# NOAA-GFDL/GRTCODE

Measured on AMD Instinct MI355X. Metric: columns/sec (60-layer, 1 cm⁻¹ LBL, LW+SW), higher is better.
Workload: dtype f64

## Files before the change

### grtcode_amd/csrc/grt_kernels.h

```cpp
#ifndef GRT_KERNELS_H_
#define GRT_KERNELS_H_

#include <stddef.h>
#include <stdint.h>

#ifdef __cplusplus
extern "C" {
#endif

#define GRT_MAX_ISO 18
#define GRT_MAX_SLOTS 53
#define GRT_MAX_TABLES 32

typedef struct GrtLineStore
{
    uint64_t n;
    double const *v0;
    double const *s0;
    float const *yair;
    float const *yself;
    float const *en;
    float const *nexp;
    float const *delta;
    uint8_t const *iso;
// ... 33 lines not shown
    GrtLineStore lines;
    GrtColumnLayout lay;
    double const *colstate;
    double const *tables;
    double const *h2o_tables;
    double w0, wres;
    uint64_t nw;
    int ncol;
    double *tau;
    uint64_t tau_col_stride;
    int tile;
    int nslice;
    int fast;
    float *gmom;
    uint64_t gmom_stride;
    int halo;
    int rcap;
    int tree_levels;
    int mom_terms;
    int profile_tag;
    int near_block;
    int deterministic;
    unsigned long long *probe;
    int direct_near;
    int tile_phase, tile_nphase;
    uint32_t const *tile_ranges;
    int lean;
    uint32_t const *tile_items;
    uint32_t n_items;
    GrtTableSpans spans;
    int *radius_table;
    int skip_tables;
    int narrow;
} GrtGasOpticsArgs;

typedef struct GrtContinua
{
    double const *colstate;
    uint64_t stride, off_cont, off_h2o;
    double const *tables;
    double const *h2o_tables;
    int num_tables, has_h2o_ctm;
    GrtTableSpans spans;
} GrtContinua;
int grt_launch_add_continua(void *stream, GrtContinua const *c, int num_layers, int ncol, uint64_t nw,
                            double *tau_gas, uint64_t col_stride);


int grt_launch_gas_optics(void *stream, GrtGasOpticsArgs const *a);
enum { GRT_TAG_FAR_OFFSET = 5 };
int grt_profile_begin(void *stream, int tag);
void grt_profile_end(void *stream, int slot);
int grt_launch_gas_optics_mp(void *stream, GrtGasOpticsArgs const *a);
int grt_gas_optics_mp_shape(GrtGasOpticsArgs const *a);
int grt_gas_optics_lean_shape(GrtGasOpticsArgs const *a);
void grt_work_order(unsigned nb, unsigned per_group, unsigned ngroups, unsigned b, unsigned *group, unsigned *rem);
int grt_tree_gather_by_wave(long long fsteps);
uint64_t grt_gas_optics_moment_floats(uint64_t nw, int levels, int terms);
double grt_gas_optics_moment_separation(int terms);

typedef struct GrtSweepBins
{
    double w0, wres;
    uint64_t num_wpoints, n;
    int ppb, do_interp, do_last_interp;
    double const *w;
    double *tau;
    uint64_t const *l, *r;
} GrtSweepBins;
int grt_launch_sweep_sort(void *stream, uint64_t n, int num_layers, double const *v0, double shift_max,
                          double const *lay, double const *prep, double *sorted);
int grt_launch_sweep(void *stream, int method, uint64_t n, int num_layers, double const *lines,
                     double const *ns, GrtSweepBins const *bins, double *tau);
int grt_launch_sweep_interpolate(void *stream, int num_layers, GrtSweepBins const *bins, double *tau);

int grt_launch_line_prep(void *stream, GrtGasOpticsArgs const *a, int col,
                         double *vnn, double *snn, double *gamma, double *alpha,
                         int64_t *win_s, int64_t *win_e);

int grt_launch_voigt_debug(void *stream, int fast, double w_start, uint64_t n, double wres, double center,
                           double gamma, double alpha, double *K_dev);

int grt_launch_voigt_points(void *stream, int variant, uint64_t n, double const *x_dev, double const *y_dev,
                            double *K_dev, int *cls_dev);

int grt_launch_device_math(void *stream, int op, uint64_t n, double const *a_dev, double *out0_dev, double *out1_dev);

int grt_launch_rayleigh(void *stream, int num_layers, double w0, double dw, uint64_t nw,
                        double const *n_layer_host, double *tau, double *omega, double *g);

typedef struct GrtOpticsPtrs { double const *tau[8]; double const *omega[8]; double const *g[8]; } GrtOpticsPtrs;
// ... 453 lines not shown
```

### grtcode_amd/csrc/hip/gas_optics_mp_dev.h

```cpp
#ifndef GRT_GAS_OPTICS_MP_DEV_H_
#define GRT_GAS_OPTICS_MP_DEV_H_
#include <type_traits>
#include "gas_optics_dev.h"

namespace {

constexpr int kMom = 8;
constexpr int kFarGradedMin = 64;
constexpr int kMomWide = 12;

__host__ __device__ inline double moment_separation(int terms)
{
    return terms == kMomWide ? 3.95 : 7.8;
}
constexpr size_t kLdsPerWorkgroup = 64*1024;
constexpr int kRcap = 12;
constexpr int kPowTable = 128;
constexpr int kCellLoop = 3;

template <int CTRL>
__device__ __forceinline__ float dpp_f(float v)
{
    int const b = __float_as_int(v);
    return __int_as_float(__builtin_amdgcn_update_dpp(0, b, CTRL, 0xf, 0xf, true));
// ... 133 lines not shown
    {
        float const keep = b1 ? x[i + 2] : x[i];
        float const send = b1 ? x[i] : x[i + 2];
        y[i] = keep + dpp_f<0x1B>(send);
    }
    float const keep = b0 ? y[1] : y[0];
    float const send = b0 ? y[0] : y[1];
    return keep + dpp_f<0xB1>(send);
}

constexpr int kRawCap = 128;
constexpr int kLeanListCap = 12;
constexpr int kLeanMaxP = 4;
constexpr int kLeanSlots = 16;
struct LeanTables
{
    float ps[kLeanSlots];
    float qn_m[kLeanSlots*GRT_MAX_ISO];
    float dop[kLeanSlots];
    float qn_e[kLeanSlots*GRT_MAX_ISO];
    float ptab[kPowTable];
    float p_ps[kLeanSlots];
};
static_assert(kLeanSlots*GRT_MAX_ISO > 255 && kLeanSlots*GRT_MAX_ISO + kPowTable > 255, "ps, dop and p_ps within reach of a paired read");
struct LeanRaw
{
    unsigned long long xl_mask[kWaves][kLeanListCap][kLeanMaxP];
    unsigned j[kWaves][kRawCap];
    float amp[kWaves][kRawCap];
    float delta[kWaves][kRawCap];
    unsigned idx[kWaves][kRawCap];
    unsigned xl_base[kWaves][kLeanListCap];
};

constexpr int kClasses = 3;
constexpr int kClassesSplit = 4;
constexpr int kMpQueue = 64;
constexpr int kMpQueueTree = 64;

template <int CAP, int NCLS>
struct MpQueue
{
    static constexpr int capacity = CAP;
    static constexpr int classes = NCLS;
    float amp[NCLS][kWaves][CAP];
    float xi[NCLS][kWaves][CAP];
    float y[NCLS][kWaves][CAP];
    unsigned short idx[NCLS][kWaves][CAP];
};
using MpQueueFlat = MpQueue<kMpQueue, kClassesSplit>;
using MpQueueTree = MpQueue<kMpQueueTree, kClassesSplit>;

__device__ __attribute__((noinline)) double exp_fp64_call(double x)
{
    return exp_fp64(x);
}

constexpr int binomial(int n, int k)
{
    int r = 1;
    for (int i = 1; i <= k; ++i)
    {
        r = r*(n - k + i)/i;
    }
    return r;
}
// ... 143 lines not shown
```

### grtcode_amd/csrc/hip/k_gas_optics_far.hip

```cpp
#include "gas_optics_mp_dev.h"

namespace {

__global__ __launch_bounds__(kBlock) void near_radius_kernel(GrtGasOpticsArgs a, long long fsteps_ll, int cell_shift, int ntiles)
{
    extern __shared__ __attribute__((aligned(16))) unsigned char smem[];
    double *ms_l = reinterpret_cast<double *>(smem);
    double *q_l = ms_l + 4*a.lay.num_slots;
    int const tid = threadIdx.x;
    int const layer = blockIdx.x, col = blockIdx.y;
    double const *cs = a.colstate + (uint64_t)col*a.lay.stride;
    double const *lay = cs + a.lay.off_lay + (uint64_t)layer*4;
    stage_column_state(a, cs, layer, ms_l, q_l, tid);
    __syncthreads();
    long long const nw = (long long)a.nw;
    for (int t = tid; t < ntiles; t += kBlock)
    {
        long long const c1 = ((long long)(t + 1) << cell_shift);
        bool um, cr;
        int const R = near_radius(a, lay, ms_l, (long long)t << cell_shift, c1 < nw ? c1 : nw, (int)fsteps_ll, &um, &cr);
        long long const F1 = c1 < nw ? c1 : nw;
        unsigned const tf = lean_tile_flags(a, lay, ms_l, (int)((long long)t << cell_shift), (int)F1, cr);
        a.radius_table[((uint64_t)col*a.lay.num_layers + layer)*ntiles + t] = R | (um ? 0x10000 : 0) | (cr ? 0x20000 : 0) | (int)(tf << kTileFlagsShift);
    }
}

__global__ __launch_bounds__(kBlock) void gas_optics_far_kernel(GrtGasOpticsArgs a, long long fsteps_ll, int cell_shift, int ncell)
{
    extern __shared__ __attribute__((aligned(16))) unsigned char smem[];
    int const fsteps = (int)fsteps_ll;
    double *acc = reinterpret_cast<double *>(smem);
    double *ms_l = acc + a.tile;
    double *q_l = ms_l + 4*a.lay.num_slots;
    float *mom = reinterpret_cast<float *>(q_l + GRT_MAX_ISO*a.lay.num_slots);
    float *invr = mom + (size_t)kMom*ncell;
    int *rtab = reinterpret_cast<int *>(invr + fsteps + 1);
    int const tid = threadIdx.x;
    int const layer = blockIdx.y, col = blockIdx.z;
    long long const nw = (long long)a.nw;
    long long const F0l = (long long)blockIdx.x*a.tile;
    long long const F1l = (F0l + a.tile < nw) ? F0l + a.tile : nw;
    int const F0 = (int)F0l, F1 = (int)F1l;
    double const *cs = a.colstate + (uint64_t)col*a.lay.stride;
    double const *lay = cs + a.lay.off_lay + (uint64_t)layer*4;
    double *out = a.tau + (uint64_t)col*a.tau_col_stride + (uint64_t)layer*a.nw;
    bool const own_radii = a.radius_table == nullptr || fsteps > kFarGradedMin;
    if (own_radii)
    {
        stage_column_state(a, cs, layer, ms_l, q_l, tid);
    }
    for (int i = tid; i <= fsteps; i += kBlock)
    {
        invr[i] = i > 0 ? 1.0f/(float)i : 0.f;
    }
    int const cell0 = F0 - fsteps;
    float const *gm = a.gmom + ((uint64_t)col*a.lay.num_layers + layer)*a.gmom_stride;
// ... 700 lines not shown
extern "C" size_t grt_far_lds_bytes(int tile, int ncell, int fsteps, int num_slots, int cell_shift)
{
    return far_lds_bytes(tile, ncell, fsteps, num_slots, cell_shift);
}

extern "C" size_t grt_tree_lds_bytes(int tile, int num_slots, int ntab)
{
    return tree_lds_bytes(tile, num_slots, ntab);
}

extern "C" int grt_tree_gather_tile(void)
{
    return tree_gather_tile();
}

extern "C" int grt_tree_gather_ntab(int tile, int halo)
{
    return tree_gather_ntab(tile, halo);
}

extern "C" int grt_tree_gather_by_wave(long long fsteps)
{
    return tree_gather_by_wave(fsteps) ? 1 : 0;
}

extern "C" int grt_launch_near_radius(void *stream, GrtGasOpticsArgs const *bp, long long fsteps, int shift)
{
    int const ntiles = (int)((bp->nw + ((uint64_t)1 << shift) - 1) >> shift);
    hipLaunchKernelGGL(near_radius_kernel, dim3(bp->lay.num_layers, bp->ncol), dim3(kBlock),
                       sizeof(double)*bp->lay.num_slots*(4 + GRT_MAX_ISO), (hipStream_t)stream, *bp, fsteps, shift, ntiles);
    return (int)hipGetLastError();
}

extern "C" int grt_launch_far_field(void *stream, GrtGasOpticsArgs const *bp, long long fsteps, int shift)
{
    hipStream_t const s = (hipStream_t)stream;
    GrtGasOpticsArgs b = *bp;
    if (b.tree_levels > 0)
    {
        int first_level = 1;
        while ((2 << (first_level - 1)) <= b.tile && first_level <= b.tree_levels) ++first_level;
        if (b.mom_terms == kMomWide)
        {
            launch_tree<kMomWide>(s, b, fsteps, shift, first_level);
        }
        else
        {
            launch_tree<kMom>(s, b, fsteps, shift, first_level);
        }
        return (int)hipGetLastError();
    }
    int const far_want = 512;
    int far_tile = b.tile;
    while (2*far_tile <= far_want && (uint64_t)far_tile < b.nw
           && far_lds_bytes(2*far_tile, 2*far_tile + 2*(int)fsteps, (int)fsteps, b.lay.num_slots, shift) <= kLdsPerWorkgroup)
    {
        far_tile *= 2;
    }
    b.tile = far_tile;
    unsigned const far_tiles = (unsigned)((b.nw + far_tile - 1)/far_tile);
    int const far_ncell = far_tile + 2*(int)fsteps;
    hipLaunchKernelGGL(gas_optics_far_kernel, dim3(far_tiles, b.lay.num_layers, b.ncol), dim3(kBlock),
                       far_lds_bytes(far_tile, far_ncell, (int)fsteps, b.lay.num_slots, shift), s, b, fsteps, shift, far_ncell);
    return (int)hipGetLastError();
}
```

### grtcode_amd/csrc/hip/k_gas_optics_mp.hip

```cpp
#include "gas_optics_mp_dev.h"

extern "C" size_t grt_far_lds_bytes(int tile, int ncell, int fsteps, int num_slots, int cell_shift);
extern "C" size_t grt_tree_lds_bytes(int tile, int num_slots, int ntab);
extern "C" int grt_tree_gather_tile(void);
extern "C" int grt_tree_gather_ntab(int tile, int halo);
extern "C" int grt_tree_gather_by_wave(long long fsteps);
extern "C" int grt_launch_far_field(void *stream, GrtGasOpticsArgs const *b, long long fsteps, int shift);
extern "C" int grt_launch_near_radius(void *stream, GrtGasOpticsArgs const *b, long long fsteps, int shift);

namespace {

template <int CLASS, int ONLY, bool PACKED4, typename Queue>
__device__ __forceinline__ void drain_class(double *acc, Queue const *q, int wave, int first, int count, int lane)
{
    for (int i = first + lane; i < first + count; i += 64)
    {
        float const xi = q->xi[CLASS][wave][i], y = q->y[CLASS][wave][i];
        unsigned const idx = q->idx[CLASS][wave][i];
        float const far = (idx & 0x8000u) ? (y*kRsqrpi)*__builtin_amdgcn_rcpf(fmaf(xi, xi, y*y)) : 0.f;
        double const k = voigt_near<true, ONLY, PACKED4>(xi, y) - (double)far;
        GRT_ACC_ADD(&acc[idx & 0x7fffu], (double)q->amp[CLASS][wave][i]*k);
    }
}

constexpr int kProbeWords = 24;
constexpr int kLeanP = 2;
template <bool TWO_PASS, bool TREE, int K, bool NARROW = false, bool PROBE = false, bool LEAN_LOOP = false>
__device__ __forceinline__ void mp_kernel_body(GrtGasOpticsArgs const &a, long long fsteps_ll, unsigned ngroups,
                                               int ncell, int nacc, int halo)
{
    extern __shared__ __attribute__((aligned(16))) unsigned char smem[];
    int const fsteps = (int)fsteps_ll;
    double *acc = reinterpret_cast<double *>(smem);
    using Queue = std::conditional_t<TREE, MpQueueTree, MpQueueFlat>;
    constexpr bool kSplit = Queue::classes == kClassesSplit;
    Queue *nq = reinterpret_cast<Queue *>(smem + sizeof(double)*nacc);
    long long *range = reinterpret_cast<long long *>(nq + 1);
    double *ms_l = reinterpret_cast<double *>(range + 2);
    double *q_l = ms_l + 4*a.lay.num_slots;
    double *ptab = q_l + GRT_MAX_ISO*a.lay.num_slots;
    float *mom = reinterpret_cast<float *>(ptab + kPowTable);
    float *invr = mom + (size_t)kMom*ncell;
    unsigned *occ_any = reinterpret_cast<unsigned *>(invr + 1);
    unsigned *occ_many = occ_any + (a.tile >> 5);

    int const tid = threadIdx.x;
    int const lane = tid & 63;
    int const wave = __builtin_amdgcn_readfirstlane(tid >> 6);
    WorkItem const wi = decode_work(a, ngroups);
    int const col = wi.col, layer = wi.layer, tile_idx = wi.tile_idx, slice = wi.slice;
    if (TWO_PASS && a.tile_nphase > 1 && tile_idx % a.tile_nphase != a.tile_phase)
    {
        return;
    }
    long long const nw = (long long)a.nw;
    long long const F0l = (long long)tile_idx*a.tile;
    long long const F1l = (F0l + a.tile < nw) ? F0l + a.tile : nw;
    int const F0 = (int)F0l, F1 = (int)F1l;
    unsigned long long *probe_rec = nullptr;
    unsigned pc_ring_inside = 0, pc_ring_lorentz = 0, pc_blocks = 0, pc_ring = 0, pc_near = 0, pc_momred = 0, pc_momlane = 0, pc_pre2 = 0, pc_walk = 0;
// ... 39 lines not shown
            if (tid == 0)
            {
                probe_rec[2] = nlines;
                probe_rec[3] = (unsigned long long)R | ((unsigned long long)corrected << 16) | ((unsigned long long)use_moments << 17);
                probe_rec[1] = __builtin_readcyclecounter();
            }
        }
    };
    int const cell0 = TWO_PASS ? F0 : F0 - fsteps;
    int const A0 = TWO_PASS ? F0 - halo : F0;

    double const *cs = a.colstate + (uint64_t)col*a.lay.stride;
    double const *lay = cs + a.lay.off_lay + (uint64_t)layer*4;

    for (int i = tid; i < nacc; i += kBlock)
    {
        acc[i] = 0.0;
    }
    for (int i = tid; i < kMom*ncell; i += kBlock)
    {
        mom[i] = 0.f;
    }
    if (TREE && K == kMomWide && ncell == 0)
    {
        for (int i = tid; i < 2*(a.tile >> 5); i += kBlock)
        {
            occ_any[i] = 0u;
        }
    }
    for (int i = tid; i <= fsteps && !TWO_PASS; i += kBlock)
    {
        invr[i] = i > 0 ? 1.0f/(float)i : 0.f;
    }
    stage_column_state(a, cs, layer, ms_l, q_l, tid);
    for (int i = tid; i < kPowTable; i += kBlock)
    {
        ptab[i] = exp_fp64((double)((float)i/100.f)*lay[3]);
    }
    if (TWO_PASS && a.tile_ranges != nullptr)
    {
        if (tid == 0 && a.tile_items != nullptr)
        {
            range[0] = (long long)a.tile_items[4*(uint64_t)wi.group + 1];
            range[1] = (long long)a.tile_items[4*(uint64_t)wi.group + 2];
        }
        else if (tid == 0)
        {
            uint64_t const jlo = a.tile_ranges[2*tile_idx], jhi = a.tile_ranges[2*tile_idx + 1];
            uint64_t const per = (jhi - jlo + a.nslice - 1)/a.nslice;
            uint64_t const b = jlo + per*slice;
            uint64_t e = b + per;
            if (e > jhi) e = jhi;
            range[0] = (long long)(b < jhi ? b : jhi);
            range[1] = (long long)e;
        }
    }
    else if (wave == 0)
    {
        candidate_range_wave(a, lay, F0l, F1l, TWO_PASS ? 0 : fsteps_ll, slice, range, lane);
    }
    __syncthreads();
    if constexpr (PROBE)
    {
        if (tid == 0) probe_rec[11] = __builtin_readcyclecounter();
    }
    uint64_t const jbeg = (uint64_t)range[0];
    uint64_t const jend = (uint64_t)range[1];

    float const wres_f = (float)a.wres;
    double const inv_wres = 1./a.wres;
// ... 348 lines not shown
#pragma unroll
                for (int k = kMom - 2; k >= 0; --k)
                {
                    pa = fmaf(pa, u, ma[k*ncell]);
                    pb = fmaf(pb, -u, mb[k*ncell]);
                }
                sum += (double)((pa + pb)*(u*u));
            }
            acc[i] += sum;
        }
        __syncthreads();
    }
    write_tile(a, acc, cs, col, layer, slice, F0l, F1l, tid);
    probe_finish(jend - jbeg, R, corrected, use_moments);
}

template <bool TWO_PASS, bool TREE = false, int K = kMom>
__global__ __launch_bounds__(kBlock) void gas_optics_mp_kernel(GrtGasOpticsArgs a, long long fsteps_ll, unsigned ngroups,
                                                                int ncell, int nacc, int halo)
{
    mp_kernel_body<TWO_PASS, TREE, K>(a, fsteps_ll, ngroups, ncell, nacc, halo);
}

constexpr int kMpWaves = 5;
template <bool TWO_PASS, bool TREE, int K, bool NARROW = false>
__global__ __launch_bounds__(kBlock) __attribute__((amdgpu_waves_per_eu(kMpWaves, kMpWaves)))
void gas_optics_mp_kernel_w5(GrtGasOpticsArgs a, long long fsteps_ll, unsigned ngroups, int ncell,
                             int nacc, int halo)
{
    mp_kernel_body<TWO_PASS, TREE, K, NARROW>(a, fsteps_ll, ngroups, ncell, nacc, halo);
}

constexpr int kLeanWaves = 4;
template <bool NARROW>
__global__ __launch_bounds__(kBlock) __attribute__((amdgpu_waves_per_eu(kLeanWaves, kLeanWaves)))
void gas_optics_lean_kernel(GrtGasOpticsArgs a, long long fsteps_ll, unsigned ngroups, int ncell,
                            int nacc, int halo)
{
    mp_kernel_body<true, false, kMom, NARROW, false, true>(a, fsteps_ll, ngroups, ncell, nacc, halo);
}

__global__ __launch_bounds__(kBlock)
void gas_optics_mp_probe_wide_kernel(GrtGasOpticsArgs a, long long fsteps_ll, unsigned ngroups, int ncell,
                                     int nacc, int halo)
{
    mp_kernel_body<true, true, kMomWide, false, true>(a, fsteps_ll, ngroups, ncell, nacc, halo);
}

template <bool NARROW>
__global__ __launch_bounds__(kBlock) __attribute__((amdgpu_waves_per_eu(4, 4)))
void gas_optics_mp_probe_kernel(GrtGasOpticsArgs a, long long fsteps_ll, unsigned ngroups, int ncell,
                                int nacc, int halo)
{
    mp_kernel_body<true, false, kMom, NARROW, true>(a, fsteps_ll, ngroups, ncell, nacc, halo);
}

size_t lean_lds_bytes(int num_slots)
{
    (void)num_slots;
    return 16 + sizeof(LeanTables) + sizeof(LeanRaw);
}

size_t mp_lds_bytes(int nacc, int ncell, int fsteps, int num_slots, bool tree = false, int subtree_tile = 0)
{
    size_t const main_loop = sizeof(double)*nacc + (tree ? sizeof(MpQueueTree) : sizeof(MpQueueFlat)) + 2*sizeof(long long) + sizeof(double)*(num_slots*(4 + GRT_MAX_ISO) + kPowTable)
                             + sizeof(float)*((size_t)kMom*ncell + fsteps + 1) + sizeof(unsigned)*2*((size_t)subtree_tile >> 5);
    size_t const subtree = sizeof(float)*kMomWide*((size_t)(subtree_tile >> 1) + (size_t)(subtree_tile >> 2));
    return main_loop > subtree ? main_loop : subtree;
}

int log2_exact(int v)
{
// ... 39 lines not shown
    }
    if (fsteps > 4096 || a->rcap != kRcap)
    {
        return 0;
    }
    if (a->mom_terms != 0 && a->mom_terms != kMom)
    {
        return 0;
    }
    if (a->fast == 3)
    {
        int const shift = log2_exact(a->tile);
        return shift >= 6 && a->halo == fsteps && a->mom_terms == kMom
               && mp_lds_bytes(a->tile + 2*(int)fsteps, a->tile, 0, a->lay.num_slots) <= kLdsPerWorkgroup
               && grt_far_lds_bytes(a->tile, a->tile + 2*(int)fsteps, (int)fsteps, a->lay.num_slots, shift) <= kLdsPerWorkgroup;
    }
    return mp_lds_bytes(a->tile, a->tile + 2*(int)fsteps, (int)fsteps, a->lay.num_slots) <= kLdsPerWorkgroup;
}

extern "C" int grt_gas_optics_lean_shape(GrtGasOpticsArgs const *a)
{
    int const nacc = a->tile + 2*a->halo;
    return a->fast == 3 && a->tree_levels == 0 && a->lines.lean_a != NULL && a->lines.lean_b != NULL
           && a->lines.lean_c != NULL && a->lines.lean_x != NULL && a->lay.num_slots <= kLeanSlots && a->lines.lean_w0 == a->w0 && a->lines.lean_wres == a->wres
           && a->lines.n < 0xffffffffull && a->halo >= 8 && nacc <= 4096
           && mp_lds_bytes(nacc, a->tile, 0, a->lay.num_slots) + lean_lds_bytes(a->lay.num_slots) <= kLdsPerWorkgroup;
}

extern "C" uint64_t grt_gas_optics_moment_floats(uint64_t nw, int levels, int terms)
{
    return level_offset(nw, levels + 1, terms == 0 ? kMom : terms, levels);
}

extern "C" double grt_gas_optics_moment_separation(int terms)
{
    return moment_separation(terms);
}

extern "C" int grt_launch_gas_optics_mp(void *stream, GrtGasOpticsArgs const *a)
{
    if (a->tile <= 0 || (a->tile % 64) != 0 || a->nslice < 1 || a->ncol < 1 || !grt_gas_optics_mp_shape(a) || !mp_bound(a))
    {
        return (int)hipErrorInvalidValue;
    }
    long long const fsteps = (long long)ceil((double)25.f/a->wres);
    if (a->nw > 0x7fffffffull)
    {
        return (int)hipErrorInvalidValue;
    }
    unsigned long long const tiles = (a->nw + a->tile - 1)/a->tile;
    bool const items = a->tile_items != nullptr;
    bool const tree = a->tree_levels > 0;
    if ((items && (a->fast != 3 || a->tile_ranges == nullptr || a->n_items == 0 || tree || a->deterministic || a->probe != NULL))
        || (a->lean && (a->probe != NULL || !grt_gas_optics_lean_shape(a))) || (a->narrow && (a->fast != 3 || tree))
        || (a->near_block != 0 && (a->near_block != 64 || !tree)))
    {
        return (int)hipErrorInvalidValue;
    }
    unsigned long long const ngroups = items ? a->n_items : tiles*a->nslice;
    unsigned long long const blocks = ngroups*a->lay.num_layers*a->ncol;
    if (blocks == 0 || blocks > 0x7fffffffull)
    {
        return (int)hipErrorInvalidValue;
    }
    hipStream_t const s = (hipStream_t)stream;
    if (a->fast == 3)
    {
        int const halo = a->halo;
        int const nacc = a->tile + 2*halo, shift = log2_exact(a->tile);
        if (a->ncol > 65535 || a->lay.num_layers > 65535 || (tree && a->nslice != 1))
        {
            return (int)hipErrorInvalidValue;
        }
        hipError_t e = hipMemsetAsync(a->tau, 0, sizeof(double)*a->tau_col_stride*(size_t)a->ncol, s);
        if (e == hipSuccess && a->nslice > 1)
        {
            e = hipMemsetAsync(a->gmom, 0, sizeof(float)*a->gmom_stride*a->lay.num_layers*a->ncol, s);
        }
        bool const wide = tree && a->mom_terms == kMomWide;
        if (e != hipSuccess)
        {
            return (int)e;
        }
        GrtGasOpticsArgs b = *a;
        if (!tree && b.radius_table != nullptr)
        {
            int const rc_radius = grt_launch_near_radius(stream, &b, fsteps, shift);
            if (rc_radius != 0)
            {
                return rc_radius;
            }
        }
        int slot = a->profile_tag ? grt_profile_begin(stream, a->profile_tag) : -1;
        int const ncell = (tree && a->tile > kDirectTile) ? 0 : a->tile;
        size_t lds = mp_lds_bytes(nacc, ncell, 0, a->lay.num_slots, tree, tree && ncell == 0 ? a->tile : 0);
        if (a->lean)
        {
            lds += lean_lds_bytes(a->lay.num_slots);
        }
        int const nphase = a->deterministic ? (2*halo)/a->tile + 2 : 1;
        if (a->deterministic && a->nslice != 1)
        {
            return (int)hipErrorInvalidValue;
        }
        void (*first_pass)(GrtGasOpticsArgs, long long, unsigned, int, int, int);
        if (wide && a->probe != NULL) first_pass = gas_optics_mp_probe_wide_kernel;
        else if (wide) first_pass = gas_optics_mp_kernel<true, true, kMomWide>;
        else if (tree) first_pass = gas_optics_mp_kernel_w5<true, true, kMom>;
        else if (a->probe != NULL) first_pass = a->narrow ? gas_optics_mp_probe_kernel<true> : gas_optics_mp_probe_kernel<false>;
        else if (a->lean) first_pass = a->narrow ? gas_optics_lean_kernel<true> : gas_optics_lean_kernel<false>;
        else first_pass = a->narrow ? gas_optics_mp_kernel_w5<true, false, kMom, true> : gas_optics_mp_kernel_w5<true, false, kMom>;
        for (int phase = 0; phase < nphase; ++phase)
        {
            b.tile_phase = phase;
            b.tile_nphase = nphase;
            hipLaunchKernelGGL(first_pass, dim3((unsigned)blocks), dim3(kBlock), lds, s, b, fsteps, (unsigned)ngroups,
                               ncell, nacc, halo);
        }
        if (a->profile_tag) grt_profile_end(stream, slot);
        b.nslice = 1;
        slot = a->profile_tag ? grt_profile_begin(stream, a->profile_tag + GRT_TAG_FAR_OFFSET) : -1;
        int const rc_far = grt_launch_far_field(stream, &b, fsteps, shift);
        if (a->profile_tag) grt_profile_end(stream, slot);
        return rc_far;
    }
    int const ncell = a->tile + 2*(int)fsteps;
    size_t const lds = mp_lds_bytes(a->tile, ncell, (int)fsteps, a->lay.num_slots);
    hipLaunchKernelGGL((gas_optics_mp_kernel_w5<false, false, kMom>), dim3((unsigned)blocks), dim3(kBlock), lds, s, *a, fsteps,
                       (unsigned)ngroups, ncell, a->tile, 0);
    return (int)hipGetLastError();
}
```

### grtcode_amd/csrc/hip/mp_lean_block.inc

```

    static_assert(kLeanP == 2, "the lean loop keeps the two lines of a lane in the halves of packed registers");
    constexpr int kLinesPerLane = LEAN_LOOP ? kLeanP : 1;
    [[maybe_unused]] bool lean_ok = false;
    [[maybe_unused]] LeanTables *lt = nullptr;
    [[maybe_unused]] LeanRaw *raw = nullptr;
    [[maybe_unused]] int rawcount = 0;
    [[maybe_unused]] int xcount = 0;
    [[maybe_unused]] float kh = 0.f, kl = 0.f, c2t = 0.f, pw = 0.f, pavg_f = 0.f, a_norm = 0.f, wres_v = 0.f, inv_wres_v = 0.f;
    [[maybe_unused]] unsigned tflags = 0u;
    auto uniform_flag = [](bool b) { return __builtin_amdgcn_readfirstlane((int)b) != 0; };
    if constexpr (LEAN_LOOP)
    {
        size_t const lean_off = ((size_t)(reinterpret_cast<unsigned char *>(invr + 1) - smem) + 15) & ~(size_t)15;
        lt = reinterpret_cast<LeanTables *>(smem + lean_off);
        raw = reinterpret_cast<LeanRaw *>(lt + 1);
        lean_ok = uniform_flag(a.lean != 0 && use_moments && R == 3 && fsteps >= 8 && halo >= 8
                               && a.lines.lean_a != nullptr);
        if (lean_ok)
        {
            for (int i = tid; i < a.lay.num_slots; i += kBlock)
            {
                lt->ps[i] = (float)ms_l[4*i];
                lt->p_ps[i] = (float)ms_l[4*i + 1];
                lt->dop[i] = (float)(((double)0.83255461115f/(double)kSqrln2)*ms_l[4*i + 3]);
            }
            for (int i = tid; i < a.lay.num_slots*GRT_MAX_ISO; i += kBlock)
            {
                double const v = q_l[i]*ms_l[(i/GRT_MAX_ISO)*4 + 2];
                int e = 0;
                double const m = frexp(v, &e);
                bool const ok = v > 0. && v < 1e300;
                lt->qn_m[i] = ok ? (float)(2.*m) : 0.f;
                lt->qn_e[i] = ok ? (float)(e - 1 - GRT_LEAN_S0_SHIFT) : 0.f;
            }
            for (int i = tid; i < kPowTable; i += kBlock)
            {
                lt->ptab[i] = (float)ptab[i];
            }
            __syncthreads();
            double const kTd = ((double)(-1.4387686f)*1.4426950408889634)*lay[2];
            kh = (float)kTd;
            kl = (float)(kTd - (double)kh);
            c2t = (float)((double)(-1.4387686f)*lay[2]);
            pw = (float)(lay[0]*inv_wres);
            pavg_f = (float)lay[0];
            a_norm = (float)(1./(3.14159265358979323846*a.wres));
            wres_v = wres_f;
            inv_wres_v = inv_wres_f;
            asm volatile("" : "+v"(kh), "+v"(kl), "+v"(c2t), "+v"(pw), "+v"(pavg_f), "+v"(a_norm), "+v"(wres_v), "+v"(inv_wres_v));
            unsigned const tf = tile_flags_known ? tile_flags : lean_tile_flags(a, lay, ms_l, F0, F1, corrected);
            tflags = (unsigned)__builtin_amdgcn_readfirstlane((int)tf);
        }
    }

    uint64_t const jal = lean_ok ? (jbeg & ~(uint64_t)1) : jbeg;
    uint64_t const walk_first = a.deterministic ? (wave == 0 ? jal : jend) : jal + (uint64_t)wave*64*kLinesPerLane;
    unsigned const walk_stride = (a.deterministic ? 64u : (unsigned)kBlock)*kLinesPerLane;

    [[maybe_unused]] auto drain_raw = [&](int const first, int const count)
    {
        if constexpr (LEAN_LOOP)
        {
            bool const on = lane < count;
            int const i = first + (on ? lane : 0);
            unsigned const packed = raw->idx[wave][i];
            unsigned const j = raw->j[wave][i];
            int const idx = (int)(packed & 4095u);
            int const c = idx + A0 - ((int)((packed >> 12) & 15u) - 3);
            double2 const lx = reinterpret_cast<double2 const *>(a.lines.lean_x)[j];
            float const yair = __int_as_float(__double2loint(lx.y)), yself = __int_as_float(__double2hiint(lx.y));
            double const *ms = ms_l + ((packed >> 16) & 63u)*4;
            double const wnoadj = lx.x + (double)raw->delta[wave][i]*lay[0];
            int const s = c - fsteps < 0 ? 0 : c - fsteps;
            LineWidths const lw = reference_widths(ptab[(packed >> 22) & 127u], yair, yself, ms, wnoadj);
            float const repwid = lw.repwid, y = lw.y;
            double const dwno = (double)s*a.wres + a.w0;
            float const xr = voigt_x(dwno, idx + A0 - s, a.wres, wnoadj, repwid);
            int const cls = on ? voigt_class<true, kSplit>(xr, y) : -1;
            queue_push(cls, raw->amp[wave][i]*(kRsqrpi*repwid), xr, y, (unsigned short)idx);
        }
    };
// ... 450 lines not shown
```

### grtcode_amd/csrc/host/grt_gas_launch.c

```c
#include <math.h>
#include <stdlib.h>
#include <string.h>
#include "grt_internal.h"
#include "../grt_work_order.h"

void grt_work_order(unsigned nb, unsigned per_group, unsigned ngroups, unsigned b, unsigned *group, unsigned *rem)
{
    grt_work_order_map(nb, per_group, ngroups, b, group, rem);
}

#define TREE_MIN_FSTEPS 200
#define ITEM_LINES 10000u

typedef struct LaunchPlan
{
    GrtGasOpticsArgs a;
    int tables;
    int items;
    double pmax;
    size_t moment_bytes;
    size_t radius_bytes;
    uint64_t probe_words;
} LaunchPlan;

static void auto_tune(GasOptics_t const *go, int ncol, int moments, int *tile, int *nslice)
{
    GrtGasOpticsImpl const *im = impl_of(go);
    uint64_t const nw = go->grid.n;
    double const per_cell = nw > 0 ? (double)im->store.n/(double)nw : 0.;
    int t = im->tile;
    if (t == 0)
    {
        int want = moments == 2 ? 256 : (moments ? 512 : 1024);
        while (moments == 2 && want > (ncol == 1 ? 128 : 64) && per_cell*(double)(want/2) >= 6000.
               && ((nw + want - 1)/want)*(uint64_t)go->num_layers*(uint64_t)ncol < 16384)
        {
            want >>= 1;
        }
        t = nw >= (uint64_t)want ? want : (int)(((nw + 63)/64)*64);
        if (moments == 2)
        {
            while (t & (t - 1))
            {
                t += 64;
            }
        }
    }
    int ns = im->nslice;
    if (ns == 0)
    {
        uint64_t const blocks = ((nw + t - 1)/t)*(uint64_t)go->num_layers*(uint64_t)ncol;
        double const per_tile = per_cell*(double)t;
        ns = 1;
        while (blocks*ns < 16384 && ns < 16 && per_tile/(double)(2*ns) >= 8000.)
// ... 242 lines not shown
            }
            a->gmom_stride = grt_gas_optics_moment_floats(a->nw, a->tree_levels, a->mom_terms);
        }
        if (!grt_gas_optics_mp_shape(a))
        {
            a->fast = im->fast == 3 ? 1 : 2;
            a->tree_levels = 0;
            a->mom_terms = 0;
            a->rcap = 12;
            if (a->fast == 1)
            {
                auto_tune(go, ncol, 1, &a->tile, &a->nslice);
                if (!grt_gas_optics_mp_shape(a))
                {
                    a->fast = 2;
                }
            }
        }
    }
    if (a->fast != 1 && a->fast != 3)
    {
        auto_tune(go, ncol, 0, &a->tile, &a->nslice);
    }
    a->direct_near = a->fast == 1 || a->fast == 3;
    uint64_t const tiles = (a->nw + (uint64_t)a->tile - 1)/(uint64_t)a->tile;
    if (a->fast == 3)
    {
        char const *lean = getenv("GRT_LEAN");
        a->lean = !(lean != NULL && lean[0] == '0') && grt_gas_optics_lean_shape(a);
        a->narrow = a->tree_levels == 0 && a->w0 + (double)a->nw*a->wres <= 4000.;
        a->near_block = a->tree_levels > 0 && grt_tree_gather_by_wave(fsteps) ? 64 : 0;
        p->moment_bytes = sizeof(float)*(size_t)a->gmom_stride*(size_t)go->num_layers;
        p->radius_bytes = a->tree_levels == 0 ? sizeof(int)*(size_t)tiles*(size_t)go->num_layers : 0;
        if (a->tree_levels == 0 || a->mom_terms == 12)
        {
            p->probe_words = 24*tiles*(uint64_t)a->nslice*(uint64_t)go->num_layers;
        }
        p->tables = im->sorted_v0_h != NULL && im->store.n > 0 && im->store.n < 0xffffffffull;
        for (int c = 0; c < ncol && p->tables && im->colstate_h != NULL; ++c)
        {
            double const *lay = im->colstate_h + (size_t)c*im->layout.stride + im->layout.off_lay;
            for (int i = 0; i < go->num_layers; ++i)
            {
                p->pmax = fabs(lay[(size_t)i*4]) > p->pmax ? fabs(lay[(size_t)i*4]) : p->pmax;
            }
        }
        char const *env = getenv("GRT_TILE_ITEMS");
        p->items = p->tables && im->nslice == 0 && a->tree_levels == 0 && !grt_deterministic()
                   && !(env != NULL && env[0] == '0') && tiles*(uint64_t)go->num_layers*(uint64_t)ncol < 16384;
    }
    if (grt_deterministic())
    {
        a->deterministic = 1;
        a->nslice = 1;
    }
}

static int grow(GasOptics_t *go, void **buf, size_t *have, size_t need)
{
    if (need > *have)
    {
        GRT_TRY(grt_dev_free(go->device, *buf));
        *buf = NULL;
        *have = 0;
        GRT_TRY(grt_dev_alloc(go->device, buf, need));
        *have = need;
    }
    return GRTCODE_SUCCESS;
}

static int bind(GasOptics_t *go, LaunchPlan const *p, int c0, int ncol, double *tau, uint64_t tau_col_stride,
                GrtGasOpticsArgs *a)
{
    GrtGasOpticsImpl *im = impl_of(go);
    *a = p->a;
    a->ncol = ncol;
    a->colstate = im->colstate_d + (size_t)c0*im->layout.stride;
    a->tau = tau + (size_t)c0*tau_col_stride;
    a->tau_col_stride = tau_col_stride;
    if (p->moment_bytes > 0)
    {
        GRT_TRY(grow(go, (void **)&im->gmom, &im->gmom_bytes, p->moment_bytes*(size_t)ncol));
        a->gmom = im->gmom;
    }
    if (p->radius_bytes > 0)
    {
        GRT_TRY(grow(go, (void **)&im->radius_table, &im->radius_bytes, p->radius_bytes*(size_t)ncol));
        a->radius_table = im->radius_table;
    }
    if (im->probe != NULL && p->probe_words > 0 && p->probe_words*(uint64_t)ncol <= im->probe_words)
    {
        a->probe = im->probe;
        a->lean = 0;
    }
    if (p->tables)
    {
        GRT_TRY(tile_tables(go, a, p->pmax));
        a->tile_ranges = im->tile_ranges_d;
        if (p->items && a->probe == NULL && im->n_items > 0)
        {
            a->tile_items = im->tile_items_d;
            a->n_items = im->n_items;
            a->nslice = im->items_cut > 1 ? 2 : 1;
        }
    }
    return GRTCODE_SUCCESS;
}

static int launch_sweep_columns(GasOptics_t *go, int ncol, double *tau_dev, uint64_t tau_col_stride)
{
    GrtGasOpticsImpl *im = impl_of(go);
    void *s = grt_dev_stream(go->device);
    int const L = go->num_layers;
    uint64_t nmax = 0;
    for (int sl = 0; sl < go->num_molecules; ++sl)
    {
        if (im->mstore[sl].n > nmax) nmax = im->mstore[sl].n;
    }
    if (nmax > 0 && im->sweep_scratch == NULL)
    {
        GRT_TRY(grt_dev_alloc(go->device, (void **)&im->sweep_scratch, sizeof(double)*8*(size_t)L*nmax));
// ... 130 lines not shown
```

### grtcode_amd/csrc/host/grt_gas_optics.c

```c
#include <math.h>
#include <stdio.h>
#include <stdlib.h>
#include <string.h>
#include "grt_internal.h"
#include "grt_molecule_table.h"

static double const MIN_CUTOFF = 1.;
static double const MAX_CUTOFF = 50.;
static double const DEFAULT_CUTOFF = 25.;

static char const *const cfc_names[NUM_CFCS] = {
    "CFC-11", "CFC-12", "CFC-113", "CFC-114", "CFC-115", "HCFC-22", "HCFC-141b", "HCFC-142b",
    "HFC-23", "HFC-125", "HFC-134a", "HFC-143a", "HFC-152a", "HFC-227ea", "HFC-245fa", "CCl4",
    "C2F6", "CF4", "CH2Cl2", "NF3", "SF6"};

int grt_load_table_on_grid(char const *path, int expect_cols, SpectralGrid_t const *grid, fp_t *out)
{
    int rows = 0, cols = 0;
    char **tok = NULL;
    GRT_TRY(parse_csv(path, &rows, &cols, 1, &tok));
    int rc = GRTCODE_SUCCESS;
    fp_t *vals = malloc(sizeof(fp_t)*(size_t)rows*(size_t)cols);
    for (int i = 0; i < rows*cols; ++i)
    {
// ... 162 lines not shown
        if (told != im->fast)
        {
            told = im->fast;
            GRT_INFO("Line kernel form %d (%s); GRT_GAS_OPTICS_FAST=0 or grt_gas_optics_tune selects the reference's operation order.",
                     im->fast, im->fast == 0 ? "reference operation order, tau within 1e-11"
                               : "fused arithmetic, tau within 2e-6 of each layer's maximum, sums in the scheduler's order");
        }
    }
    size_t const V = (size_t)num_levels;
    go->x = calloc(NUM_MOLS*V, sizeof(fp_t));
    go->x_cfc = calloc(NUM_CFCS*V, sizeof(fp_t));
    go->x_cia = calloc(NUM_CIAS*V, sizeof(fp_t));
    GRT_TRY(grt_dev_alloc(go->device, (void **)&im->lin_tables, sizeof(double)*GRT_MAX_TABLES*grid->n));
    im->store_dirty = 1;
    GRT_TRY(inittips_d());
    GRT_INFO("Gas optics on device %d: %d levels, %zu grid points.", go->device, num_levels, (size_t)grid->n);
    return GRTCODE_SUCCESS;
}

EXTERN int destroy_gas_optics(GasOptics_t * const gas_optics)
{
    GRT_REQUIRE_PTR(gas_optics);
    GrtGasOpticsImpl *im = impl_of(gas_optics);
    if (im != NULL)
    {
        for (int i = 0; i < NUM_MOLS; ++i)
        {
            grt_free_host_lines(&im->host[i]);
        }
        GRT_TRY(grt_free_line_store(gas_optics));
        GRT_TRY(grt_dev_free(gas_optics->device, im->bins_block));
        GRT_TRY(grt_dev_free(gas_optics->device, im->gmom));
        GRT_TRY(grt_dev_free(gas_optics->device, im->radius_table));
        GRT_TRY(grt_dev_free(gas_optics->device, im->h2o_tables));
        GRT_TRY(grt_dev_free(gas_optics->device, im->lin_tables));
        GRT_TRY(grt_dev_free(gas_optics->device, im->colstate_d));
        GRT_TRY(grt_host_free_pinned(im->colstate_h));
        GRT_TRY(grt_dev_event_destroy(gas_optics->device, &im->colstate_uploaded));
        free(im);
    }
    free(gas_optics->h2o_cc.coefs);
    free(gas_optics->x);
    free(gas_optics->x_cfc);
    free(gas_optics->x_cia);
    gas_optics->impl = NULL;
    gas_optics->x = gas_optics->x_cfc = gas_optics->x_cia = NULL;
    gas_optics->h2o_cc.coefs = NULL;
    return GRTCODE_SUCCESS;
}

static int register_molecule(GasOptics_t *go, int molecule_id, GrtHostLines *lines, double w0, double wn)
{
    GrtGasOpticsImpl *im = impl_of(go);
    int const index = go->num_molecules;
    Molecule_t *mol = &go->mols[index];
    memset(mol, 0, sizeof(*mol));
    mol->id = molecule_id;
    mol->device = go->device;
    snprintf(mol->name, MOL_NAME_LEN, "%s", grt_molecule_table[molecule_id - 1].name);
    mol->mass = grt_molecule_table[molecule_id - 1].molar_mass;
    mol->mass /= 6.023e23;
    mol->num_isotopologues = grt_molecule_table[molecule_id - 1].num_iso;
    mol->line_params.num_lines = lines->n;
    mol->line_params.device = go->device;
    im->host[index] = *lines;
    memset(lines, 0, sizeof(*lines));
// ... 772 lines not shown
```

### grtcode_amd/csrc/host/grt_internal.h

```cpp
#ifndef GRT_INTERNAL_H_
#define GRT_INTERNAL_H_

#include <stddef.h>
#include <stdint.h>
#include "grtcode_hip_api.h"
#include "grt_ext.h"
#include "../grt_kernels.h"

void grt_err_begin(int code, char const *file, int line, char const *fmt, ...);
void grt_err_frame(char const *file, int line);
void grt_log(int level, char const *file, int line, char const *fmt, ...);

#define GRT_FAIL(code, ...) \
    do { grt_err_begin((code), __FILE__, __LINE__, __VA_ARGS__); return (code); } while (0)

#define GRT_TRY(expr) \
    do { int rc_ = (expr); if (rc_ != GRTCODE_SUCCESS) { grt_err_frame(__FILE__, __LINE__); return rc_; } } while (0)

#define GRT_REQUIRE_PTR(p) \
    do { if ((p) == NULL) GRT_FAIL(GRTCODE_NULL_ERR, "null pointer for argument '%s'.", #p); } while (0)

#define GRT_REQUIRE_RANGE(v, lo, hi) \
    do { double v_ = (double)(v), lo_ = (double)(lo), hi_ = (double)(hi); \
         if (v_ != v_) GRT_FAIL(GRTCODE_INVALID_ERR, "input value (%e) is Nan.", v_); \
// ... 45 lines not shown

typedef struct GrtHostLines
{
    uint64_t n;
    double *v0, *s0;
    float *yair, *yself, *en, *nexp, *delta;
    uint8_t *iso;
} GrtHostLines;

typedef struct GrtGasOpticsImpl
{
    GrtHostLines host[NUM_MOLS];
    int store_dirty;
    unsigned long store_tips_generation;
    GrtLineStore store;
    void *store_block;
    double *sorted_v0_h;
    uint32_t *tile_ranges_d;
    int tr_tile;
    uint64_t tr_tiles;
    double tr_pbound;
    uint32_t *tile_items_d;
    uint32_t *tile_items_h, *tile_ranges_h;
    uint32_t n_items;
    int items_cut;
    GrtLineStore mstore[NUM_MOLS];
    void *mstore_block[NUM_MOLS];
    double *sweep_scratch;
    void *bins_block;
    float *gmom;
    size_t gmom_bytes;
    int *radius_table;
    size_t radius_bytes;
    size_t scratch_cap_bytes;
    long long last_launch[8];
    double *h2o_tables;
    double *lin_tables;
    int num_lin;
    int lin_kind[GRT_MAX_TABLES];
    int lin_ref[GRT_MAX_TABLES];
    GrtTableSpans spans;
    int defer_tables;
    GrtColumnLayout layout;
    int layout_cols;
    double *colstate_h;
    void *colstate_uploaded;
    double *colstate_d;
    int tile, nslice, fast;
    int profile_tag;
    unsigned long long *probe;
    uint64_t probe_words;
} GrtGasOpticsImpl;
static inline GrtGasOpticsImpl *impl_of(GasOptics_t const *go) { return (GrtGasOpticsImpl *)go->impl; }

#define GRT_PRIVATE __attribute__((visibility("hidden")))

static inline size_t grt_align256(size_t x) { return (x + 255) & ~(size_t)255; }

int grt_gas_optics_prepare(GasOptics_t *go, int ncol);
int grt_gas_optics_wait_staging(GasOptics_t *go);
GRT_PRIVATE int grt_gas_optics_stage_column(GasOptics_t *go, fp_t const *p_mb, fp_t const *t);
GRT_PRIVATE int grt_gas_optics_upload_states(GasOptics_t *go, int ncol);
int grt_column_state(GasOptics_t const *go, fp_t const *p_mb, fp_t const *t,
                     fp_t const *x_mol , fp_t const *x_cfc ,
                     fp_t const *x_cia , double *dst);
int grt_gas_optics_defer_tables(GasOptics_t *go, int on);
// ... 30 lines not shown
```

Baseline: 647.7.

## Precompute per-layer state and lean tables once in a separate kernel

Adds a layer_tables_kernel that builds each (column, layer)'s staged column state, pow table, lean float tables and uniforms once and writes them as an image to global memory. The multi-pass and lean gas-optics kernels then copy this image into LDS instead of recomputing exp and frexp work in every spectral tile block. This trades redundant per-block arithmetic for an extra launch and global-memory reads. It is enabled by default for non-tree paths and can be turned off with GRT_LAYER_TABLES=0.

```diff
diff --git a/grtcode_amd/csrc/grt_kernels.h b/grtcode_amd/csrc/grt_kernels.h
--- a/grtcode_amd/csrc/grt_kernels.h
+++ b/grtcode_amd/csrc/grt_kernels.h
@@ -89,6 +89,7 @@
     int *radius_table;
     int skip_tables;
     int narrow;
+    unsigned char *layer_tables;
 } GrtGasOpticsArgs;
 
 typedef struct GrtContinua
@@ -114,6 +115,7 @@
 void grt_work_order(unsigned nb, unsigned per_group, unsigned ngroups, unsigned b, unsigned *group, unsigned *rem);
 int grt_tree_gather_by_wave(long long fsteps);
 uint64_t grt_gas_optics_moment_floats(uint64_t nw, int levels, int terms);
+size_t grt_gas_optics_layer_image_bytes(int num_slots);
 double grt_gas_optics_moment_separation(int terms);
 
 typedef struct GrtSweepBins
diff --git a/grtcode_amd/csrc/hip/gas_optics_mp_dev.h b/grtcode_amd/csrc/hip/gas_optics_mp_dev.h
--- a/grtcode_amd/csrc/hip/gas_optics_mp_dev.h
+++ b/grtcode_amd/csrc/hip/gas_optics_mp_dev.h
@@ -189,6 +189,68 @@
     unsigned idx[kWaves][kRawCap];
     unsigned xl_base[kWaves][kLeanListCap];
 };
+
+constexpr int kLeanUniforms = 8;
+static_assert((4 + GRT_MAX_ISO) % 2 == 0 && kPowTable % 2 == 0 && sizeof(LeanTables) % 16 == 0 && kLeanUniforms % 4 == 0,
+              "the parts of a layer image are copied in 16-byte pieces");
+
+__host__ __device__ inline size_t layer_state_doubles(int num_slots)
+{
+    return (size_t)num_slots*(4 + GRT_MAX_ISO) + kPowTable;
+}
+
+__host__ __device__ inline size_t layer_image_bytes(int num_slots)
+{
+    return sizeof(double)*layer_state_doubles(num_slots) + sizeof(LeanTables) + sizeof(float)*kLeanUniforms;
+}
+
+__device__ __forceinline__ void build_layer_state(GrtGasOpticsArgs const &a, double const *cs, double const *lay, int layer,
+                                                  double *ms_l, double *q_l, double *ptab, int tid)
+{
+    stage_column_state(a, cs, layer, ms_l, q_l, tid);
+    for (int i = tid; i < kPowTable; i += kBlock)
+    {
+        ptab[i] = exp_fp64((double)((float)i/100.f)*lay[3]);
+    }
+}
+
+__device__ __forceinline__ void build_lean_tables(GrtGasOpticsArgs const &a, double const *ms_l, double const *q_l,
+                                                  double const *ptab, LeanTables *lt, int tid)
+{
+    for (int i = tid; i < a.lay.num_slots; i += kBlock)
+    {
+        lt->ps[i] = (float)ms_l[4*i];
+        lt->p_ps[i] = (float)ms_l[4*i + 1];
+        lt->dop[i] = (float)(((double)0.83255461115f/(double)kSqrln2)*ms_l[4*i + 3]);
+    }
+    for (int i = tid; i < a.lay.num_slots*GRT_MAX_ISO; i += kBlock)
+    {
+        double const v = q_l[i]*ms_l[(i/GRT_MAX_ISO)*4 + 2];
+        int e = 0;
+        double const m = frexp(v, &e);
+        bool const ok = v > 0. && v < 1e300;
+        lt->qn_m[i] = ok ? (float)(2.*m) : 0.f;
+        lt->qn_e[i] = ok ? (float)(e - 1 - GRT_LEAN_S0_SHIFT) : 0.f;
+    }
+    for (int i = tid; i < kPowTable; i += kBlock)
+    {
+        lt->ptab[i] = (float)ptab[i];
+    }
+}
+
+__device__ __forceinline__ void lean_uniforms(GrtGasOpticsArgs const &a, double const *lay, float (&u)[kLeanUniforms])
+{
+    double const inv_wres = 1./a.wres;
+    double const kTd = ((double)(-1.4387686f)*1.4426950408889634)*lay[2];
+    u[0] = (float)kTd;
+    u[1] = (float)(kTd - (double)u[0]);
+    u[2] = (float)((double)(-1.4387686f)*lay[2]);
+    u[3] = (float)(lay[0]*inv_wres);
+    u[4] = (float)lay[0];
+    u[5] = (float)(1./(3.14159265358979323846*a.wres));
+    u[6] = (float)a.wres;
+    u[7] = (float)inv_wres;
+}
 
 constexpr int kClasses = 3;
 constexpr int kClassesSplit = 4;
diff --git a/grtcode_amd/csrc/hip/k_gas_optics_far.hip b/grtcode_amd/csrc/hip/k_gas_optics_far.hip
--- a/grtcode_amd/csrc/hip/k_gas_optics_far.hip
+++ b/grtcode_amd/csrc/hip/k_gas_optics_far.hip
@@ -22,6 +22,48 @@
         long long const F1 = c1 < nw ? c1 : nw;
         unsigned const tf = lean_tile_flags(a, lay, ms_l, (int)((long long)t << cell_shift), (int)F1, cr);
         a.radius_table[((uint64_t)col*a.lay.num_layers + layer)*ntiles + t] = R | (um ? 0x10000 : 0) | (cr ? 0x20000 : 0) | (int)(tf << kTileFlagsShift);
+    }
+}
+
+__global__ __launch_bounds__(kBlock) void layer_tables_kernel(GrtGasOpticsArgs a)
+{
+    extern __shared__ __attribute__((aligned(16))) unsigned char smem[];
+    size_t const nstate = layer_state_doubles(a.lay.num_slots);
+    double *ms_l = reinterpret_cast<double *>(smem);
+    double *q_l = ms_l + 4*a.lay.num_slots;
+    double *ptab = q_l + GRT_MAX_ISO*a.lay.num_slots;
+    LeanTables *lt = reinterpret_cast<LeanTables *>(ms_l + nstate);
+    float *un = reinterpret_cast<float *>(lt + 1);
+    int const tid = threadIdx.x;
+    int const layer = blockIdx.x, col = blockIdx.y;
+    double const *cs = a.colstate + (uint64_t)col*a.lay.stride;
+    double const *lay = cs + a.lay.off_lay + (uint64_t)layer*4;
+    build_layer_state(a, cs, lay, layer, ms_l, q_l, ptab, tid);
+    for (int i = tid; i < (int)((sizeof(LeanTables) + sizeof(float)*kLeanUniforms)/sizeof(float)); i += kBlock)
+    {
+        reinterpret_cast<float *>(lt)[i] = 0.f;
+    }
+    __syncthreads();
+    if (a.lay.num_slots <= kLeanSlots)
+    {
+        build_lean_tables(a, ms_l, q_l, ptab, lt, tid);
+        if (tid == 0)
+        {
+            float u[kLeanUniforms];
+            lean_uniforms(a, lay, u);
+#pragma unroll
+            for (int i = 0; i < kLeanUniforms; ++i)
+            {
+                un[i] = u[i];
+            }
+        }
+    }
+    __syncthreads();
+    size_t const bytes = layer_image_bytes(a.lay.num_slots);
+    float4 *out = reinterpret_cast<float4 *>(a.layer_tables + ((uint64_t)col*a.lay.num_layers + layer)*bytes);
+    for (int i = tid; i < (int)(bytes/16); i += kBlock)
+    {
+        out[i] = reinterpret_cast<float4 const *>(smem)[i];
     }
 }
 
@@ -788,6 +830,17 @@
     return (int)hipGetLastError();
 }
 
+extern "C" int grt_launch_layer_tables(void *stream, GrtGasOpticsArgs const *bp)
+{
+    size_t const lds = layer_image_bytes(bp->lay.num_slots);
+    if (lds > kLdsPerWorkgroup || bp->lay.num_layers > 65535 || bp->ncol > 65535)
+    {
+        return (int)hipErrorInvalidValue;
+    }
+    hipLaunchKernelGGL(layer_tables_kernel, dim3(bp->lay.num_layers, bp->ncol), dim3(kBlock), lds, (hipStream_t)stream, *bp);
+    return (int)hipGetLastError();
+}
+
 extern "C" int grt_launch_far_field(void *stream, GrtGasOpticsArgs const *bp, long long fsteps, int shift)
 {
     hipStream_t const s = (hipStream_t)stream;
diff --git a/grtcode_amd/csrc/hip/k_gas_optics_mp.hip b/grtcode_amd/csrc/hip/k_gas_optics_mp.hip
--- a/grtcode_amd/csrc/hip/k_gas_optics_mp.hip
+++ b/grtcode_amd/csrc/hip/k_gas_optics_mp.hip
@@ -7,6 +7,7 @@
 extern "C" int grt_tree_gather_by_wave(long long fsteps);
 extern "C" int grt_launch_far_field(void *stream, GrtGasOpticsArgs const *b, long long fsteps, int shift);
 extern "C" int grt_launch_near_radius(void *stream, GrtGasOpticsArgs const *b, long long fsteps, int shift);
+extern "C" int grt_launch_layer_tables(void *stream, GrtGasOpticsArgs const *b);
 
 namespace {
 
@@ -25,7 +26,7 @@
 
 constexpr int kProbeWords = 24;
 constexpr int kLeanP = 2;
-template <bool TWO_PASS, bool TREE, int K, bool NARROW = false, bool PROBE = false, bool LEAN_LOOP = false>
+template <bool TWO_PASS, bool TREE, int K, bool NARROW = false, bool PROBE = false, bool LEAN_LOOP = false, bool IMAGE = false>
 __device__ __forceinline__ void mp_kernel_body(GrtGasOpticsArgs const &a, long long fsteps_ll, unsigned ngroups,
                                                int ncell, int nacc, int halo)
 {
@@ -131,10 +132,36 @@
     {
         invr[i] = i > 0 ? 1.0f/(float)i : 0.f;
     }
-    stage_column_state(a, cs, layer, ms_l, q_l, tid);
-    for (int i = tid; i < kPowTable; i += kBlock)
-    {
-        ptab[i] = exp_fp64((double)((float)i/100.f)*lay[3]);
+    bool const have_image = LEAN_LOOP ? IMAGE : (TWO_PASS && !TREE && a.layer_tables != nullptr);
+    [[maybe_unused]] unsigned char const *image = nullptr;
+    [[maybe_unused]] float4 lean_u0 = make_float4(0.f, 0.f, 0.f, 0.f), lean_u1 = lean_u0;
+    if (have_image)
+    {
+        image = a.layer_tables + ((uint64_t)col*a.lay.num_layers + layer)*layer_image_bytes(a.lay.num_slots);
+        double2 const *src = reinterpret_cast<double2 const *>(image);
+        int const npair = (int)(layer_state_doubles(a.lay.num_slots) >> 1);
+        for (int i = tid; i < npair; i += kBlock)
+        {
+            double2 const v = src[i];
+            ms_l[2*i] = v.x;
+            ms_l[2*i + 1] = v.y;
+        }
+        if constexpr (LEAN_LOOP)
+        {
+            size_t const lean_off = ((size_t)(reinterpret_cast<unsigned char *>(invr + 1) - smem) + 15) & ~(size_t)15;
+            float4 const *src4 = reinterpret_cast<float4 const *>(image + sizeof(double)*layer_state_doubles(a.lay.num_slots));
+            float4 *dst4 = reinterpret_cast<float4 *>(smem + lean_off);
+            for (int i = tid; i < (int)(sizeof(LeanTables)/16); i += kBlock)
+            {
+                dst4[i] = src4[i];
+            }
+            lean_u0 = src4[sizeof(LeanTables)/16];
+            lean_u1 = src4[sizeof(LeanTables)/16 + 1];
+        }
+    }
+    else
+    {
+        build_layer_state(a, cs, lay, layer, ms_l, q_l, ptab, tid);
     }
     if (TWO_PASS && a.tile_ranges != nullptr)
     {
@@ -549,12 +576,12 @@
 }
 
 constexpr int kLeanWaves = 4;
-template <bool NARROW>
+template <bool NARROW, bool IMAGE>
 __global__ __launch_bounds__(kBlock) __attribute__((amdgpu_waves_per_eu(kLeanWaves, kLeanWaves)))
 void gas_optics_lean_kernel(GrtGasOpticsArgs a, long long fsteps_ll, unsigned ngroups, int ncell,
                             int nacc, int halo)
 {
-    mp_kernel_body<true, false, kMom, NARROW, false, true>(a, fsteps_ll, ngroups, ncell, nacc, halo);
+    mp_kernel_body<true, false, kMom, NARROW, false, true, IMAGE>(a, fsteps_ll, ngroups, ncell, nacc, halo);
 }
 
 __global__ __launch_bounds__(kBlock)
@@ -660,6 +687,11 @@
     return level_offset(nw, levels + 1, terms == 0 ? kMom : terms, levels);
 }
 
+extern "C" size_t grt_gas_optics_layer_image_bytes(int num_slots)
+{
+    return layer_image_bytes(num_slots);
+}
+
 extern "C" double grt_gas_optics_moment_separation(int terms)
 {
     return moment_separation(terms);
@@ -719,6 +751,18 @@
                 return rc_radius;
             }
         }
+        if (tree)
+        {
+            b.layer_tables = nullptr;
+        }
+        if (b.layer_tables != nullptr)
+        {
+            int const rc_tables = grt_launch_layer_tables(stream, &b);
+            if (rc_tables != 0)
+            {
+                return rc_tables;
+            }
+        }
         int slot = a->profile_tag ? grt_profile_begin(stream, a->profile_tag) : -1;
         int const ncell = (tree && a->tile > kDirectTile) ? 0 : a->tile;
         size_t lds = mp_lds_bytes(nacc, ncell, 0, a->lay.num_slots, tree, tree && ncell == 0 ? a->tile : 0);
@@ -736,7 +780,8 @@
         else if (wide) first_pass = gas_optics_mp_kernel<true, true, kMomWide>;
         else if (tree) first_pass = gas_optics_mp_kernel_w5<true, true, kMom>;
         else if (a->probe != NULL) first_pass = a->narrow ? gas_optics_mp_probe_kernel<true> : gas_optics_mp_probe_kernel<false>;
-        else if (a->lean) first_pass = a->narrow ? gas_optics_lean_kernel<true> : gas_optics_lean_kernel<false>;
+        else if (a->lean && b.layer_tables != nullptr) first_pass = a->narrow ? gas_optics_lean_kernel<true, true> : gas_optics_lean_kernel<false, true>;
+        else if (a->lean) first_pass = a->narrow ? gas_optics_lean_kernel<true, false> : gas_optics_lean_kernel<false, false>;
         else first_pass = a->narrow ? gas_optics_mp_kernel_w5<true, false, kMom, true> : gas_optics_mp_kernel_w5<true, false, kMom>;
         for (int phase = 0; phase < nphase; ++phase)
         {
diff --git a/grtcode_amd/csrc/hip/mp_lean_block.inc b/grtcode_amd/csrc/hip/mp_lean_block.inc
--- a/grtcode_amd/csrc/hip/mp_lean_block.inc
+++ b/grtcode_amd/csrc/hip/mp_lean_block.inc
@@ -18,35 +18,27 @@
                                && a.lines.lean_a != nullptr);
         if (lean_ok)
         {
-            for (int i = tid; i < a.lay.num_slots; i += kBlock)
-            {
-                lt->ps[i] = (float)ms_l[4*i];
-                lt->p_ps[i] = (float)ms_l[4*i + 1];
-                lt->dop[i] = (float)(((double)0.83255461115f/(double)kSqrln2)*ms_l[4*i + 3]);
-            }
-            for (int i = tid; i < a.lay.num_slots*GRT_MAX_ISO; i += kBlock)
-            {
-                double const v = q_l[i]*ms_l[(i/GRT_MAX_ISO)*4 + 2];
-                int e = 0;
-                double const m = frexp(v, &e);
-                bool const ok = v > 0. && v < 1e300;
-                lt->qn_m[i] = ok ? (float)(2.*m) : 0.f;
-                lt->qn_e[i] = ok ? (float)(e - 1 - GRT_LEAN_S0_SHIFT) : 0.f;
-            }
-            for (int i = tid; i < kPowTable; i += kBlock)
-            {
-                lt->ptab[i] = (float)ptab[i];
-            }
-            __syncthreads();
-            double const kTd = ((double)(-1.4387686f)*1.4426950408889634)*lay[2];
-            kh = (float)kTd;
-            kl = (float)(kTd - (double)kh);
-            c2t = (float)((double)(-1.4387686f)*lay[2]);
-            pw = (float)(lay[0]*inv_wres);
-            pavg_f = (float)lay[0];
-            a_norm = (float)(1./(3.14159265358979323846*a.wres));
-            wres_v = wres_f;
-            inv_wres_v = inv_wres_f;
+            float un[kLeanUniforms];
+            if constexpr (IMAGE)
+            {
+                float4 const u0 = lean_u0, u1 = lean_u1;
+                un[0] = u0.x; un[1] = u0.y; un[2] = u0.z; un[3] = u0.w;
+                un[4] = u1.x; un[5] = u1.y; un[6] = u1.z; un[7] = u1.w;
+            }
+            else
+            {
+                build_lean_tables(a, ms_l, q_l, ptab, lt, tid);
+                __syncthreads();
+                lean_uniforms(a, lay, un);
+            }
+            kh = un[0];
+            kl = un[1];
+            c2t = un[2];
+            pw = un[3];
+            pavg_f = un[4];
+            a_norm = un[5];
+            wres_v = un[6];
+            inv_wres_v = un[7];
             asm volatile("" : "+v"(kh), "+v"(kl), "+v"(c2t), "+v"(pw), "+v"(pavg_f), "+v"(a_norm), "+v"(wres_v), "+v"(inv_wres_v));
             unsigned const tf = tile_flags_known ? tile_flags : lean_tile_flags(a, lay, ms_l, F0, F1, corrected);
             tflags = (unsigned)__builtin_amdgcn_readfirstlane((int)tf);
diff --git a/grtcode_amd/csrc/host/grt_gas_launch.c b/grtcode_amd/csrc/host/grt_gas_launch.c
--- a/grtcode_amd/csrc/host/grt_gas_launch.c
+++ b/grtcode_amd/csrc/host/grt_gas_launch.c
@@ -20,6 +20,7 @@
     double pmax;
     size_t moment_bytes;
     size_t radius_bytes;
+    size_t image_bytes;
     uint64_t probe_words;
 } LaunchPlan;
 
@@ -328,6 +329,9 @@
         a->near_block = a->tree_levels > 0 && grt_tree_gather_by_wave(fsteps) ? 64 : 0;
         p->moment_bytes = sizeof(float)*(size_t)a->gmom_stride*(size_t)go->num_layers;
         p->radius_bytes = a->tree_levels == 0 ? sizeof(int)*(size_t)tiles*(size_t)go->num_layers : 0;
+        char const *images = getenv("GRT_LAYER_TABLES");
+        p->image_bytes = a->tree_levels == 0 && !(images != NULL && images[0] == '0')
+                         ? grt_gas_optics_layer_image_bytes(a->lay.num_slots)*(size_t)go->num_layers : 0;
         if (a->tree_levels == 0 || a->mom_terms == 12)
         {
             p->probe_words = 24*tiles*(uint64_t)a->nslice*(uint64_t)go->num_layers;
@@ -383,6 +387,11 @@
     {
         GRT_TRY(grow(go, (void **)&im->radius_table, &im->radius_bytes, p->radius_bytes*(size_t)ncol));
         a->radius_table = im->radius_table;
+    }
+    if (p->image_bytes > 0)
+    {
+        GRT_TRY(grow(go, (void **)&im->layer_tables, &im->layer_tables_bytes, p->image_bytes*(size_t)ncol));
+        a->layer_tables = im->layer_tables;
     }
     if (im->probe != NULL && p->probe_words > 0 && p->probe_words*(uint64_t)ncol <= im->probe_words)
     {
diff --git a/grtcode_amd/csrc/host/grt_gas_optics.c b/grtcode_amd/csrc/host/grt_gas_optics.c
--- a/grtcode_amd/csrc/host/grt_gas_optics.c
+++ b/grtcode_amd/csrc/host/grt_gas_optics.c
@@ -218,6 +218,7 @@
         GRT_TRY(grt_dev_free(gas_optics->device, im->bins_block));
         GRT_TRY(grt_dev_free(gas_optics->device, im->gmom));
         GRT_TRY(grt_dev_free(gas_optics->device, im->radius_table));
+        GRT_TRY(grt_dev_free(gas_optics->device, im->layer_tables));
         GRT_TRY(grt_dev_free(gas_optics->device, im->h2o_tables));
         GRT_TRY(grt_dev_free(gas_optics->device, im->lin_tables));
         GRT_TRY(grt_dev_free(gas_optics->device, im->colstate_d));
diff --git a/grtcode_amd/csrc/host/grt_internal.h b/grtcode_amd/csrc/host/grt_internal.h
--- a/grtcode_amd/csrc/host/grt_internal.h
+++ b/grtcode_amd/csrc/host/grt_internal.h
@@ -101,6 +101,8 @@
     size_t gmom_bytes;
     int *radius_table;
     size_t radius_bytes;
+    unsigned char *layer_tables;
+    size_t layer_tables_bytes;
     size_t scratch_cap_bytes;
     long long last_launch[8];
     double *h2o_tables;
```

Measured after the change: 651.4 (median of 6 runs). No clear change (+0.6%).
